# cartographer-project/point_cloud_viewer

Measured on NVIDIA H100. Metric: build_octree Mpoints/sec, higher is better.
Workload: dtype f64

## Files before the change

point_cloud_viewer_b200/csrc/build_host.hpp:

```cpp
#pragma once
#include <algorithm>
#include <chrono>
#include <cmath>
#include <cstdint>
#include <cstdio>
#include <cstdlib>
#include <cstring>
#include <stdexcept>
#include <string>
#include <vector>

#include "chain.h"

namespace pcv {

typedef unsigned __int128 u128;

struct PointsView {
    const double* x;
    const double* y;
    const double* z;
    uint64_t stride;
    const uint8_t* rgb;
    const float* intensity;
// ... 84 lines not shown
    uint64_t arena_used;
    uint32_t deepest_level, pad;
    uint32_t nleaves, place_tiles;
    uint64_t out_points, xyz_bytes, algo_xyz;
    PassState pass[kMaxPasses + 1];
};
enum : int32_t { kErrHistMismatch = 1, kErrTooDeep = 2, kErrCapacity = 3 };

struct ShardSpec {
    int k = 0;
    const uint64_t* counts = nullptr;
    PCV_HD static size_t level_offset(int level) { return (((size_t)1 << (3 * level)) - 8) / 7; }
    uint64_t count_at(int level, uint64_t index) const { return counts[level_offset(level) + index]; }
};

struct PlanRun {
    uint32_t nodes, actives, tiles, chunks;
    uint64_t next_pts, arena_pts;
};

struct IngestArgs {
    PointsView pts;
    void* rec_out;
    uint32_t* col_out;
    uint8_t* dig_out;
    int G0;
    bool wide;
    uint32_t ntiles;
    LevelTable lv;
    double root_min[3];
};

struct PassArgs {
    int pass, level, G, nbins;
    int Gn;
    bool wide;
    bool rec_has_col;
    bool holes;
    const RemoteBufs* remote;
    const float* int_in;
    double e1, e2, ry2, eb, eh, ryh;
    int enc1, enc2, ench, fast;
    const void* rec_in;
    void* rec_next;
    void* arena;
    const uint32_t* col_in;
    uint32_t* col_next;
    uint32_t* col_arena;
    const uint8_t* dig_in;
    uint8_t* dig_next;
    BuildState* st;
    const ActiveDesc* active;
    ActiveDesc* active_next;
    const ChunkDesc* chunks;
    ChunkDesc* chunks_next;
    uint32_t* tile_active;
    uint32_t* tile_counts;
    uint32_t* chunk_sums;
    uint64_t* node_bins;
    BucketDesc* buckets;
    PlanRun* plan_runs;
    DevNode* nodes;
    int32_t* children;
    uint32_t cap_active, cap_nodes, cap_tiles, cap_chunks;
    uint64_t max_points;
    double resolution;
    int shard_k;
    const uint64_t* shard_counts;
    LevelTable lv;
};

struct PlaceArgs {
    bool wide;
    PointsView pts;
    const void* arena;
    const uint32_t* col_arena;
    int fast;
    const DNode* d_nodes;
    const uint32_t* d_leaf_tile_begin;
    const uint32_t* d_leaf_node;
    uint32_t nleaves;
    uint32_t ntiles;
    uint64_t npoints, xyz_bytes;
    uint32_t prefetch_tiles = 0;
    uint8_t* out_xyz;
    uint8_t* out_rgb;
    float* out_intensity;
    uint32_t* out_src;
};

PCV_HD uint32_t upper_index(const uint32_t* begin, size_t stride_words, uint32_t n, uint32_t b) {
    uint32_t lo = 0, hi = n;
    while (hi - lo > 1) {
        const uint32_t mid = (lo + hi) >> 1;
        if (begin[(size_t)mid * stride_words] <= b)
            lo = mid;
        else
            hi = mid;
    }
    return lo;
}
PCV_HD TileDesc tile_of(const ActiveDesc* active, uint32_t nactive, uint32_t b) {
    const uint32_t i = upper_index(&active[0].tile_begin, sizeof(ActiveDesc) / 4, nactive, b);
    const ActiveDesc& act = active[i];
    const uint64_t o = (uint64_t)(b - act.tile_begin) * kTilePoints;
    const uint64_t rem = act.count - o;
    return TileDesc{act.start + o, (uint32_t)(rem < kTilePoints ? rem : kTilePoints), i};
}
PCV_HD LeafTile leaf_tile_of(const PlaceArgs& a, uint32_t b) {
    const uint32_t l = upper_index(a.d_leaf_tile_begin, 1, a.nleaves, b);
    const uint32_t node = a.d_leaf_node[l];
    const DNode& nd = a.d_nodes[node];
    const uint64_t o = (uint64_t)(b - a.d_leaf_tile_begin[l]) * kPlaceTile;
    const uint64_t rem = nd.count - o;
    return LeafTile{nd.arena_off + o, o, node, (uint32_t)(rem < kPlaceTile ? rem : kPlaceTile)};
}

template <bool EMIT>
PCV_HD void plan_active(const PassArgs& a, uint32_t ai, PlanRun& run, int32_t& err, uint32_t& deepest) {
    const ActiveDesc act = a.active[ai];
    const DevNode pn = a.nodes[act.node];
    const uint64_t* nb = a.node_bins + (size_t)ai * a.nbins;
    BucketDesc* bk = a.buckets + (size_t)ai * a.nbins;
    const int w = a.nbins / 8;
    uint32_t nlocal = 0;
    if (!EMIT) {
        uint64_t total = 0;
        for (int b = 0; b < a.nbins; ++b) total += nb[b];
        if (total != act.count) err = kErrHistMismatch;
    }
    auto route = [&](uint32_t node_index, int level, const double m[3], uint64_t cnt, bool split, int b0, int b1, int keep) {
        BucketDesc bd{};
        bd.b0 = (uint16_t)b0;
        bd.b1 = (uint16_t)b1;
        bd.keep = (uint8_t)keep;
        if (split) {
            bd.kind = 0;
            bd.dest = run.next_pts;
            const uint32_t nt = (uint32_t)((cnt + kTilePoints - 1) / kTilePoints);
            const uint32_t nc = (nt + kChunkTiles - 1) / kChunkTiles;
            if (EMIT && run.actives < a.cap_active && run.chunks + nc <= a.cap_chunks) {
                ActiveDesc& na = a.active_next[run.actives];
                na.m[0] = m[0], na.m[1] = m[1], na.m[2] = m[2];
                na.e = a.lv.edge[level];
                na.start = run.next_pts;
                na.count = cnt;
                na.chunk_begin = run.chunks;
                na.nchunks = nc;
                na.tile_begin = run.tiles;
                na.node = node_index;
                for (uint32_t o = 0, c = 0; o < nt; o += kChunkTiles, ++c)
                    a.chunks_next[run.chunks + c] = ChunkDesc{run.tiles + o, (nt - o < kChunkTiles ? nt - o : kChunkTiles), run.actives, o == 0 ? 1u : 0u};
            }
            run.actives += 1;
            run.tiles += nt;
            run.chunks += nc;
            run.next_pts += cnt;
        } else {
            bd.kind = 1;
            bd.dest = run.arena_pts;
            if (EMIT && node_index < a.cap_nodes) a.nodes[node_index].arena_off = run.arena_pts;
            run.arena_pts += cnt;
            if (a.holes) run.next_pts += cnt;
            if ((uint32_t)level > deepest) deepest = (uint32_t)level;
        }
        if (EMIT) bk[nlocal] = bd;
        ++nlocal;
// ... 637 lines not shown
    r.enc = lv.enc[0];
    r.count = total;
    nodes.push_back(r);
    for (size_t i = 0; i < nodes.size(); ++i) {
        if (nodes[i].level >= k - 1) continue;
        for (int c = 0; c < 8; ++c) {
            const HNode p = nodes[i];
            const uint64_t cidx = ((uint64_t)p.index << 3) + (uint64_t)c;
            const uint64_t cnt = sp.count_at(p.level + 1, cidx);
            if (cnt == 0) continue;
            HNode x{};
            x.level = p.level + 1;
            x.index = cidx;
            x.parent = (int)i;
            for (int q = 0; q < 8; ++q) x.child[q] = -1;
            x.count = cnt;
            x.e = lv.edge[x.level];
            x.m[0] = (c & 4) ? p.m[0] + x.e : p.m[0];
            x.m[1] = (c & 2) ? p.m[1] + x.e : p.m[1];
            x.m[2] = (c & 1) ? p.m[2] + x.e : p.m[2];
            x.enc = lv.enc[x.level];
            nodes[i].child[c] = (int)nodes.size();
            nodes.push_back(x);
        }
    }
    std::vector<uint64_t> unit_off(nodes.size() * 8, 0);
    for (size_t i = nodes.size(); i-- > 0;) {
        HNode& x = nodes[i];
        uint64_t off = 0;
        if (x.level == k - 1) {
            for (int c = 0; c < 8; ++c) {
                unit_off[i * 8 + c] = off;
                off += (unit_nsub[((uint64_t)x.index << 3) + (uint64_t)c] + 7) / 8;
            }
        } else {
            for (int c = 0; c < 8; ++c) {
                if (x.child[c] < 0) continue;
                nodes[x.child[c]].off_in_parent = off;
                off += (nodes[x.child[c]].n_sub + 7) / 8;
            }
        }
        x.n_sub = off;
    }
    for (auto& x : nodes) x.final_count = x.parent < 0 ? x.n_sub : x.n_sub - (x.n_sub + 7) / 8;
    R.sorted.resize(nodes.size());
    for (size_t i = 0; i < nodes.size(); ++i) R.sorted[i] = (int)i;
    std::sort(R.sorted.begin(), R.sorted.end(), [&](int a, int b) {
        if (nodes[a].level != nodes[b].level) return nodes[a].level < nodes[b].level;
        return nodes[a].index < nodes[b].index;
    });
    uint64_t poff = 0, boff = 0, arena_total = 0;
    for (int i : R.sorted) {
        HNode& x = nodes[i];
        x.out_point_off = poff;
        boff = (boff + 15) & ~15ull;
        x.out_xyz_off = boff;
        poff += x.final_count;
        boff += x.final_count * 3 * (uint64_t)enc_bytes(x.enc);
        if (x.level == k - 1) {
            x.arena_off = arena_total;
            arena_total += x.n_sub;
        }
    }
    if (arena_total != npoints || poff != npoints) throw BuildError(-1, "top assembly: gathered point count does not match the unit sizes");
    R.xyz_bytes = boff;

    const int cenc = lv.enc[k - 1], bpc = enc_bytes(cenc);
    const size_t rec_bytes = wide ? sizeof(RecW) : sizeof(RecN);
    std::vector<uint8_t> recs((size_t)npoints * rec_bytes);
    std::vector<uint32_t> cols(npoints);
    for (uint64_t i = 0; i < npoints; ++i) {
        uint64_t c[3] = {0, 0, 0};
        for (int a = 0; a < 3; ++a) std::memcpy(&c[a], xyz + (i * 3 + a) * bpc, (size_t)bpc);
        if (wide) {
            RecW w{{c[0], c[1], c[2]}, (uint32_t)i, 0};
            std::memcpy(&recs[i * rec_bytes], &w, sizeof w);
        } else {
            RecN w{{(uint32_t)c[0], (uint32_t)c[1], (uint32_t)c[2]}, (uint32_t)i};
            std::memcpy(&recs[i * rec_bytes], &w, sizeof w);
        }
        cols[i] = (uint32_t)rgb[3 * i] | ((uint32_t)rgb[3 * i + 1] << 8) | ((uint32_t)rgb[3 * i + 2] << 16);
    }
    std::vector<void*> scratch;
    auto up = [&](const void* h, size_t bytes) {
        void* d = be.dmalloc(bytes ? bytes : 16);
        scratch.push_back(d);
        if (bytes) be.h2d(d, h, bytes);
        return d;
    };
    std::vector<DNode> dn(nodes.size());
    std::vector<uint32_t> leaf_tile_begin, leaf_node;
    uint32_t nplace_tiles = 0;
    for (size_t i = 0; i < nodes.size(); ++i) {
        const HNode& x = nodes[i];
        DNode& d = dn[i];
        for (int a = 0; a < 3; ++a) d.m[a] = x.m[a];
        d.e = x.e;
        d.ry = 1.0 / x.e;
        d.off_in_parent = x.off_in_parent;
        d.out_point_off = x.out_point_off;
        d.out_xyz_off = x.out_xyz_off;
        d.arena_off = x.arena_off;
        d.count = x.level == k - 1 ? x.n_sub : 0;
        d.parent = x.parent;
        d.enc = x.enc;
        if (x.level == k - 1 && x.n_sub) {
            leaf_tile_begin.push_back(nplace_tiles);
            leaf_node.push_back((uint32_t)i);
            nplace_tiles += (uint32_t)((x.n_sub + kPlaceTile - 1) / kPlaceTile);
        }
    }
    leaf_tile_begin.push_back(nplace_tiles);
    PlaceArgs pl{};
    pl.wide = wide;
    pl.pts = PointsView{nullptr, nullptr, nullptr, 1, nullptr, intensity ? (const float*)up(intensity, (size_t)npoints * 4) : nullptr, npoints};
    pl.arena = up(recs.data(), recs.size());
    pl.col_arena = (const uint32_t*)up(cols.data(), cols.size() * 4);
    pl.fast = lv.fast;
    pl.d_nodes = (const DNode*)up(dn.data(), dn.size() * sizeof(DNode));
    pl.d_leaf_tile_begin = (const uint32_t*)up(leaf_tile_begin.data(), leaf_tile_begin.size() * 4);
    pl.d_leaf_node = (const uint32_t*)up(leaf_node.data(), leaf_node.size() * 4);
    pl.nleaves = (uint32_t)leaf_node.size();
    pl.ntiles = nplace_tiles;
    pl.npoints = npoints;
    pl.xyz_bytes = boff;
    R.d_xyz = (uint8_t*)be.dmalloc(boff + 32);
    R.d_rgb = (uint8_t*)be.dmalloc(std::max<uint64_t>(npoints * 3, 16));
    R.d_src = (uint32_t*)be.dmalloc(std::max<uint64_t>(npoints * 4, 16));
    R.d_intensity = intensity ? (float*)be.dmalloc(std::max<uint64_t>(npoints * 4, 16)) : nullptr;
    pl.out_xyz = R.d_xyz;
    pl.out_rgb = R.d_rgb;
    pl.out_intensity = R.d_intensity;
    pl.out_src = R.d_src;
    be.place(pl);
    for (void* p : scratch) be.dfree(p);
    return R;
}

}
```

point_cloud_viewer_b200/csrc/kernels_build.cuh:

```cuda
#pragma once
#include <cuda_runtime.h>

#include <map>
#include <type_traits>
#include <unordered_map>

#include "build_host.hpp"
#include "chain_device.cuh"

namespace pcv {

#define PCV_CUDA_CHECK(x)                                                                            \
    do {                                                                                             \
        cudaError_t e_ = (x);                                                                        \
        if (e_ != cudaSuccess) throw ::pcv::BuildError(-2, std::string("CUDA: ") + cudaGetErrorString(e_) + " at " #x); \
    } while (0)

__device__ __forceinline__ double warp_min(double v) {
#pragma unroll
    for (int o = 16; o > 0; o >>= 1) v = fmin(v, __shfl_xor_sync(0xffffffffu, v, o));
    return v;
}
__device__ __forceinline__ double warp_max(double v) {
#pragma unroll
    for (int o = 16; o > 0; o >>= 1) v = fmax(v, __shfl_xor_sync(0xffffffffu, v, o));
    return v;
}

__global__ void __launch_bounds__(256) k_bbox(PointsView p, double* __restrict__ partial) {
    double mn[3] = {INFINITY, INFINITY, INFINITY}, mx[3] = {-INFINITY, -INFINITY, -INFINITY};
    const uint64_t step = (uint64_t)gridDim.x * blockDim.x;
    uint64_t i = (uint64_t)blockIdx.x * blockDim.x + threadIdx.x;
    const uint64_t s = p.stride;
    for (; i + 3 * step < p.n; i += 4 * step) {
        double vx[4], vy[4], vz[4];
#pragma unroll
        for (int u = 0; u < 4; ++u) {
            vx[u] = __ldg(p.x + (i + u * step) * s);
            vy[u] = __ldg(p.y + (i + u * step) * s);
            vz[u] = __ldg(p.z + (i + u * step) * s);
        }
#pragma unroll
        for (int u = 0; u < 4; ++u) {
            mn[0] = fmin(mn[0], vx[u]);
            mx[0] = fmax(mx[0], vx[u]);
            mn[1] = fmin(mn[1], vy[u]);
            mx[1] = fmax(mx[1], vy[u]);
            mn[2] = fmin(mn[2], vz[u]);
            mx[2] = fmax(mx[2], vz[u]);
        }
    }
    for (; i < p.n; i += step) {
        double x = __ldg(p.x + i * s), y = __ldg(p.y + i * s), z = __ldg(p.z + i * s);
        mn[0] = fmin(mn[0], x);
        mx[0] = fmax(mx[0], x);
        mn[1] = fmin(mn[1], y);
        mx[1] = fmax(mx[1], y);
        mn[2] = fmin(mn[2], z);
        mx[2] = fmax(mx[2], z);
    }
    __shared__ double sh[8][6];
    const int w = threadIdx.x >> 5, l = threadIdx.x & 31;
#pragma unroll
    for (int a = 0; a < 3; ++a) {
        double lo = warp_min(mn[a]), hi = warp_max(mx[a]);
        if (l == 0) {
            sh[w][a] = lo;
            sh[w][3 + a] = hi;
        }
    }
    __syncthreads();
    if (threadIdx.x < 6) {
        double v = sh[0][threadIdx.x];
        for (int k = 1; k < 8; ++k) v = threadIdx.x < 3 ? fmin(v, sh[k][threadIdx.x]) : fmax(v, sh[k][threadIdx.x]);
        partial[blockIdx.x * 6 + threadIdx.x] = v;
    }
}

__device__ __forceinline__ void l2_prefetch(const void* p, uint64_t bytes) {
    const uintptr_t b = (reinterpret_cast<uintptr_t>(p) + 15) & ~(uintptr_t)15;
    const uintptr_t e = (reinterpret_cast<uintptr_t>(p) + bytes) & ~(uintptr_t)15;
    if (e > b) asm volatile("cp.async.bulk.prefetch.L2.global [%0], %1;" ::"l"(b), "r"((uint32_t)(e - b)) : "memory");
}
template <bool WIDE>
struct RecT;
template <>
struct RecT<false> {
    typedef RecN type;
};
template <>
struct RecT<true> {
    typedef RecW type;
};

template <bool WIDE>
__device__ __forceinline__ void load_rec(const void* base, uint64_t i, uint64_t c[3], uint32_t& idx) {
    if (WIDE) {
        const ulonglong2* p = reinterpret_cast<const ulonglong2*>(base) + 2 * i;
        const ulonglong2 v0 = __ldg(p), v1 = __ldg(p + 1);
        c[0] = v0.x;
        c[1] = v0.y;
        c[2] = v1.x;
        idx = (uint32_t)v1.y;
    } else {
        const uint4 v = __ldg(reinterpret_cast<const uint4*>(base) + i);
        c[0] = v.x;
        c[1] = v.y;
        c[2] = v.z;
        idx = v.w;
    }
}
template <bool WIDE>
__device__ __forceinline__ void store_rec(void* base, uint64_t i, const uint64_t c[3], uint32_t idx) {
    if (WIDE) {
        ulonglong2 v0, v1;
        v0.x = c[0];
        v0.y = c[1];
        v1.x = c[2];
        v1.y = idx;
        ulonglong2* p = reinterpret_cast<ulonglong2*>(base) + 2 * i;
        p[0] = v0;
        p[1] = v1;
    } else {
        uint4 v;
        v.x = (uint32_t)c[0];
        v.y = (uint32_t)c[1];
        v.z = (uint32_t)c[2];
        v.w = idx;
        reinterpret_cast<uint4*>(base)[i] = v;
    }
}

__device__ __forceinline__ uint32_t smem_u32(const void* p) { return (uint32_t)__cvta_generic_to_shared(p); }
__device__ __forceinline__ void mbar_init(uint64_t* bar, uint32_t count) {
    asm volatile("mbarrier.init.shared.b64 [%0], %1;" ::"r"(smem_u32(bar)), "r"(count) : "memory");
    asm volatile("fence.mbarrier_init.release.cluster;" ::: "memory");
}
__device__ __forceinline__ void mbar_expect_tx(uint64_t* bar, uint32_t bytes) {
    asm volatile("mbarrier.arrive.expect_tx.release.cta.shared::cta.b64 _, [%0], %1;" ::"r"(smem_u32(bar)), "r"(bytes) : "memory");
}
__device__ __forceinline__ void tma_bulk_load(void* smem_dst, const void* gmem_src, uint32_t bytes, uint64_t* bar) {
    asm volatile("cp.async.bulk.shared::cluster.global.mbarrier::complete_tx::bytes [%0], [%1], %2, [%3];" ::"r"(smem_u32(smem_dst)), "l"(gmem_src), "r"(bytes),
                 "r"(smem_u32(bar))
                 : "memory");
}
__device__ __forceinline__ void mbar_wait(uint64_t* bar, uint32_t parity) {
    uint32_t done = 0;
    while (!done) {
        asm volatile(
            "{\n\t.reg .pred P;\n\t"
            "mbarrier.try_wait.parity.shared::cta.b64 P, [%1], %2;\n\t"
            "selp.b32 %0, 1, 0, P;\n\t}"
            : "=r"(done)
            : "r"(smem_u32(bar)), "r"(parity)
            : "memory");
    }
}

template <bool WIDE>
__device__ __forceinline__ void smem_load_rec(const unsigned char* srec, uint32_t i, uint64_t c[3], uint32_t& idx) {
    if (WIDE) {
        const ulonglong2* p = reinterpret_cast<const ulonglong2*>(srec) + 2 * (size_t)i;
        const ulonglong2 v0 = p[0], v1 = p[1];
        c[0] = v0.x, c[1] = v0.y, c[2] = v1.x, idx = (uint32_t)v1.y;
    } else {
        const uint4 v = reinterpret_cast<const uint4*>(srec)[i];
        c[0] = v.x, c[1] = v.y, c[2] = v.z, idx = v.w;
    }
}

constexpr int kIngestThreads = 256;
constexpr size_t kRgbStage = (size_t)kTilePoints * 3 + 32;

template <bool WIDE, int FAST, int kIngestBatch>
__device__ __forceinline__ unsigned ingest_tile(const IngestArgs& a, uint64_t start, uint32_t count, const uint32_t* scol) {
    unsigned bad = 0;
    const double e0 = a.lv.edge[0], e1 = a.lv.edge[1], ry1 = a.lv.ry[1];
    for (uint32_t i0 = threadIdx.x; i0 < count; i0 += kIngestThreads * kIngestBatch) {
      double qq[kIngestBatch][3];
#pragma unroll
      for (int u = 0; u < kIngestBatch; ++u) {
          const uint32_t i = i0 + u * kIngestThreads;
          const uint64_t g = start + (i < count ? i : i0);
          qq[u][0] = __ldcg(a.pts.x + g * a.pts.stride);
          qq[u][1] = __ldcg(a.pts.y + g * a.pts.stride);
          qq[u][2] = __ldcg(a.pts.z + g * a.pts.stride);
      }
#pragma unroll
      for (int u = 0; u < kIngestBatch; ++u) {
        const uint32_t i = i0 + u * kIngestThreads;
        if (i >= count) break;
        const uint64_t g = start + i;
        double q[3] = {qq[u][0], qq[u][1], qq[u][2]}, m[3] = {a.root_min[0], a.root_min[1], a.root_min[2]};
        if (FAST == 2) bad |= input_bad(q[0]) | input_bad(q[1]) | input_bad(q[2]);
// ... 674 lines not shown
                        pb.dig = (unsigned long long)rb.dig_next + (unsigned long long)first;
                        const long long slot0 = leaf ? first + (long long)(bd.dest >> 32) - (long long)(uint32_t)bd.dest : first;
                        PassBucketExt bx;
                        bx.inten = (unsigned long long)rb.intensity + (unsigned long long)(slot0 * 4);
                        bx.slot0 = (uint32_t)slot0;
                        bx.pad = 0;
                        bext[lb] = bx;
                    } else {
                    pb.rec = (unsigned long long)(leaf ? a.arena : a.rec_next) + (unsigned long long)(first * (long long)recsz);
                    pb.col = (unsigned long long)(leaf ? a.col_arena : a.col_next) + (unsigned long long)(first * 4);
                    pb.dig = (unsigned long long)a.dig_next + (unsigned long long)first;
                    }
                    pb.start = run;
                    pb.kk = (uint32_t)bd.keep | (leaf ? 0x100u : 0u);
                    bdst[lb] = pb;
#pragma unroll
                    for (int w = 0; w < kWarps; ++w) {
                        const uint32_t c = cnt[w * nbmax + lb];
                        cnt[w * nbmax + lb] = run;
                        run += c;
                    }
                }
            }
        }
        __syncthreads();
#pragma unroll
        for (int r = 0; r < kSubRounds; ++r) {
            const uint32_t i = warp * kWarpItems + r * 32 + lane;
            const uint32_t lbv = info[r] & 0xFFFFu, rank = (info[r] >> 16) & 31u, gsize = ((info[r] >> 26) & 31u) + 1u;
            const int leader = (int)((info[r] >> 21) & 31u);
            uint32_t old = 0;
            if (lane == leader && lbv != 0xFFFFu) {
                old = cnt[warp * nbmax + lbv];
                cnt[warp * nbmax + lbv] = old + gsize;
            }
            old = __shfl_sync(0xffffffffu, old, leader);
            if (lbv != 0xFFFFu) perm[old + rank] = i | (lbv << 12);
            __syncwarp();
        }
        if (stage_next) {
            asm volatile("cp.async.wait_all;" ::: "memory");
            pass_make_desc(&descs[s ^ 1u], ntile, *snact, nact);
            pass_stage_small<WIDE>(a, descs[s ^ 1u], smem_raw + PassSmem<WIDE>::off_small + (size_t)(s ^ 1u) * PassSmem<WIDE>::small_bytes, &mbar[s ^ 1u]);
        }
        __syncthreads();
        mbar_wait(&mbar[2], it & 1u);
        if (FASTMODE == 1) {
            const unsigned bad = pass_finish<WIDE, 1, REMOTE, ENCU>(a, pt, srec, scol, sdig, perm, bdst, bext);
            if (__syncthreads_or((int)bad)) pass_finish<WIDE, 0, REMOTE, ENCU>(a, pt, srec, scol, sdig, perm, bdst, bext);
        } else {
            pass_finish<WIDE, FASTMODE, REMOTE, ENCU>(a, pt, srec, scol, sdig, perm, bdst, bext);
        }
        __syncthreads();
        if (stage_next) pass_stage_big<WIDE>(a, descs[s ^ 1u], smem_raw, &mbar[2]);
    }
}

__device__ __forceinline__ void store_code(uint8_t* p, uint64_t c, int enc) {
    if (enc == ENC_U8)
        *p = (uint8_t)c;
    else if (enc == ENC_U16)
        *reinterpret_cast<uint16_t*>(p) = (uint16_t)c;
    else if (enc == ENC_F32)
        *reinterpret_cast<uint32_t*>(p) = (uint32_t)c;
    else
        *reinterpret_cast<uint64_t*>(p) = c;
}

__device__ __forceinline__ void place_store(const PlaceArgs& a, const DNode& nd, uint64_t slot, const uint64_t c[3], uint32_t col, uint32_t idx) {
    const uint64_t dp = nd.out_point_off + slot;
    const int bpc = enc_bytes(nd.enc);
    uint8_t* px = a.out_xyz + nd.out_xyz_off + slot * 3 * (uint64_t)bpc;
    store_code(px, c[0], nd.enc);
    store_code(px + bpc, c[1], nd.enc);
    store_code(px + 2 * bpc, c[2], nd.enc);
    uint8_t* rd = a.out_rgb + 3ull * dp;
    rd[0] = (uint8_t)col;
    rd[1] = (uint8_t)(col >> 8);
    rd[2] = (uint8_t)(col >> 16);
    a.out_src[dp] = idx;
    if (a.out_intensity) a.out_intensity[dp] = __ldg(a.pts.intensity + idx);
}

template <bool WIDE, int ENC, int FAST>
__device__ __forceinline__ unsigned place_stayers(const PlaceArgs& a, const LeafTile& lt, const DNode& nd) {
    unsigned bad = 0;
    const uint32_t nst = lt.count - (lt.count + 7) / 8;
    for (uint32_t s = threadIdx.x; s < nst; s += blockDim.x) {
        const uint32_t i = 8 * (s / 7) + (s % 7) + 1;
        uint64_t c[3];
        uint32_t idx;
        load_rec<WIDE>(a.arena, lt.arena_start + i, c, idx);
        const uint32_t col = __ldg(a.col_arena + lt.arena_start + i);
#pragma unroll
        for (int k = 0; k < 3; ++k) c[k] = encode_axis<ENC, FAST>(decode_axis<ENC>(c[k], nd.m[k], nd.e), nd.m[k], nd.e, nd.ry, bad);
        if (!FAST || !bad) {
            const uint64_t j = lt.j0 + i;
            place_store(a, nd, j - (j >> 3) - 1, c, col, idx);
        }
    }
    return bad;
}

template <bool WIDE>
__device__ __forceinline__ void place_movers(const PlaceArgs& a, const LeafTile& lt, const DNode& leaf, bool all_points) {
    const uint32_t step = all_points ? 1u : 8u;
    for (uint32_t i = threadIdx.x * step; i < lt.count; i += blockDim.x * step) {
        uint64_t c[3];
        uint32_t idx;
        load_rec<WIDE>(a.arena, lt.arena_start + i, c, idx);
        const uint32_t col = __ldg(a.col_arena + lt.arena_start + i);
        uint64_t j = lt.j0 + i;
        DNode nd = leaf;
        while (nd.parent >= 0 && (j & 7) == 0) {
            const DNode P = a.d_nodes[nd.parent];
#pragma unroll
            for (int k = 0; k < 3; ++k) {
                if (a.fast) {
                    const double q = decode1_fast(c[k], nd.m[k], nd.e, nd.enc);
                    c[k] = encode1_fast(q, P.m[k], P.e, P.ry, P.enc);
                } else {
                    const double q = decode1(c[k], nd.m[k], nd.e, nd.enc);
                    c[k] = encode1(q, P.m[k], P.e, P.enc);
                }
            }
            j = nd.off_in_parent + (j >> 3);
            nd = P;
        }
        uint64_t slot = j;
        if (nd.parent >= 0) {
#pragma unroll
            for (int k = 0; k < 3; ++k) {
                if (a.fast) {
                    const double q = decode1_fast(c[k], nd.m[k], nd.e, nd.enc);
                    c[k] = encode1_fast(q, nd.m[k], nd.e, nd.ry, nd.enc);
                } else {
                    const double q = decode1(c[k], nd.m[k], nd.e, nd.enc);
                    c[k] = encode1(q, nd.m[k], nd.e, nd.enc);
                }
            }
            slot = j - (j >> 3) - 1;
        }
        place_store(a, nd, slot, c, col, idx);
    }
}

template <bool WIDE>
__global__ void __launch_bounds__(256) k_place(const __grid_constant__ PlaceArgs a) {
    const LeafTile lt = leaf_tile_of(a, blockIdx.x);
    const DNode leaf = a.d_nodes[lt.node];
    if (threadIdx.x == 32 && a.prefetch_tiles) {
        const uint64_t first = lt.arena_start + (uint64_t)a.prefetch_tiles * kPlaceTile;
        if (first < a.npoints) {
            const uint64_t cnt = min((uint64_t)kPlaceTile, a.npoints - first), rb = WIDE ? 32 : 16;
            l2_prefetch(reinterpret_cast<const unsigned char*>(a.arena) + first * rb, cnt * rb);
            l2_prefetch(a.col_arena + first, cnt * 4);
        }
    }
    const bool generic = leaf.parent < 0 || (lt.j0 & 7) != 0;
    if (generic) {
        place_movers<WIDE>(a, lt, leaf, true);
        return;
    }
    if (a.fast == 3) {
        PCV_ENC_SWITCH(leaf.enc, place_stayers<WIDE, ENC, 3>(a, lt, leaf);)
    } else if (a.fast) {
        unsigned bad = 0;
        if (a.fast == 2) {
            PCV_ENC_SWITCH(leaf.enc, bad = place_stayers<WIDE, ENC, 2>(a, lt, leaf);)
        } else {
            PCV_ENC_SWITCH(leaf.enc, bad = place_stayers<WIDE, ENC, 1>(a, lt, leaf);)
        }
        if (__syncthreads_or((int)bad)) {
            PCV_ENC_SWITCH(leaf.enc, place_stayers<WIDE, ENC, 0>(a, lt, leaf);)
        }
    } else {
        PCV_ENC_SWITCH(leaf.enc, place_stayers<WIDE, ENC, 0>(a, lt, leaf);)
    }
    place_movers<WIDE>(a, lt, leaf, false);
}

struct CudaBackend : Backend {
    cudaStream_t stream = nullptr;
    uint64_t launches = 0;
    cudaEvent_t ev[4] = {nullptr, nullptr, nullptr, nullptr};
    enum { K_BBOX = 0, K_INGEST, K_DIGHIST, K_SCAN, K_PLAN, K_PASS, K_PLACE, K_PLY, K_COUNT };
    struct KStat {
        uint64_t launches = 0, bytes = 0;
        double ms = 0;
    };
    bool profile = false;
    KStat kstat[K_COUNT];
    struct Pending {
        int k;
        cudaEvent_t e0, e1;
        uint64_t bytes;
        int pass;
    };
    std::vector<Pending> pending;
    void prof_begin(int k, uint64_t bytes, int pass = -1) {
        if (!profile) return;
        Pending p{k, nullptr, nullptr, bytes, pass};
        cudaEventCreate(&p.e0);
        cudaEventCreate(&p.e1);
        cudaEventRecord(p.e0, stream);
        pending.push_back(p);
    }
    void prof_end() {
        if (!profile) return;
        cudaEventRecord(pending.back().e1, stream);
    }
    void prof_collect() {
        for (auto& p : pending) {
            float ms = 0;
            cudaEventElapsedTime(&ms, p.e0, p.e1);
            kstat[p.k].launches++;
            kstat[p.k].ms += ms;
            kstat[p.k].bytes += p.bytes;
            cudaEventDestroy(p.e0);
            cudaEventDestroy(p.e1);
        }
        pending.clear();
    }
    void prof_reset() {
        for (auto& k : kstat) k = KStat();
    }

    explicit CudaBackend(cudaStream_t s) : stream(s) {
        for (auto& e : ev) PCV_CUDA_CHECK(cudaEventCreate(&e));
        allow_smem_all();
    }
    ~CudaBackend() override {
        cache_release();
        if (ev_back) cudaEventDestroy(ev_back);
        for (auto& b : back_chunks) cudaFreeHost(b.p);
        for (auto& e : ev)
            if (e) cudaEventDestroy(e);
        if (pin) cudaFreeHost(pin);
        if (pin_back) cudaFreeHost(pin_back);
    }
    static constexpr size_t kCacheMin = (size_t)1 << 20;
    struct CachedBlock {
        void* p;
        uint64_t seq;
    };
    std::unordered_map<void*, size_t> big_live;
    std::multimap<size_t, CachedBlock> big_free;
    size_t cached_bytes = 0, cache_cap = 0;
    uint64_t cache_seq = 0;
    void cache_release() {
        for (auto& kv : big_free) cudaFreeAsync(kv.second.p, stream);
        big_free.clear();
        cached_bytes = 0;
    }
    void cache_evict_oldest() {
        auto best = big_free.begin();
        for (auto it = big_free.begin(); it != big_free.end(); ++it)
            if (it->second.seq < best->second.seq) best = it;
        cudaFreeAsync(best->second.p, stream);
        cached_bytes -= best->first;
        big_free.erase(best);
    }
// ... 17 lines not shown
            auto it = big_free.find(bytes);
            if (it != big_free.end()) {
                p = it->second.p;
                big_free.erase(it);
                cached_bytes -= bytes;
                big_live[p] = bytes;
                return p;
            }
        }
        cudaError_t e = cudaMallocAsync(&p, bytes ? bytes : 16, stream);
        if (e == cudaErrorMemoryAllocation && !big_free.empty()) {
            cudaGetLastError();
            cache_release();
            e = cudaMallocAsync(&p, bytes ? bytes : 16, stream);
        }
        PCV_CUDA_CHECK(e);
        if (bytes >= kCacheMin) big_live[p] = bytes;
        return p;
    }
    void dfree(void* p) override {
        if (!p) return;
        auto it = big_live.find(p);
        if (it == big_live.end()) {
            cudaFreeAsync(p, stream);
            return;
        }
        if (!cache_cap) {
            size_t fr = 0, tot = 0;
            cudaMemGetInfo(&fr, &tot);
            cache_cap = tot / 2;
        }
        const size_t bytes = it->second;
        big_live.erase(it);
        big_free.emplace(bytes, CachedBlock{p, ++cache_seq});
        cached_bytes += bytes;
        while (cached_bytes > cache_cap && !big_free.empty()) cache_evict_oldest();
    }
    uint8_t* pin = nullptr;
    size_t pin_cap = 0, pin_off = 0;
    void h2d(void* d, const void* h, size_t bytes) override {
        if (bytes == 0) return;
        const size_t need = (bytes + 255) & ~(size_t)255;
        if (need > pin_cap / 2) {
            PCV_CUDA_CHECK(cudaStreamSynchronize(stream));
            if (pin) cudaFreeHost(pin);
            pin_cap = std::max<size_t>(need * 4, (size_t)64 << 20);
            PCV_CUDA_CHECK(cudaMallocHost(&pin, pin_cap));
            pin_off = 0;
        }
        if (pin_off + need > pin_cap) {
            PCV_CUDA_CHECK(cudaStreamSynchronize(stream));
            pin_off = 0;
        }
        std::memcpy(pin + pin_off, h, bytes);
        PCV_CUDA_CHECK(cudaMemcpyAsync(d, pin + pin_off, bytes, cudaMemcpyHostToDevice, stream));
        pin_off += need;
    }
    uint8_t* pin_back = nullptr;
    size_t pin_back_cap = 0;
    void d2h(void* h, const void* d, size_t bytes) override {
        if (bytes > pin_back_cap) {
            if (pin_back) cudaFreeHost(pin_back);
            pin_back_cap = std::max<size_t>(bytes * 2, (size_t)8 << 20);
            PCV_CUDA_CHECK(cudaMallocHost(&pin_back, pin_back_cap));
        }
        PCV_CUDA_CHECK(cudaMemcpyAsync(pin_back, d, bytes, cudaMemcpyDeviceToHost, stream));
        PCV_CUDA_CHECK(cudaStreamSynchronize(stream));
        std::memcpy(h, pin_back, bytes);
        pin_off = 0;
    }
    void mark(int what) override { cudaEventRecord(ev[what], stream); }

    void zero(void* d, size_t bytes) override {
        if (bytes) PCV_CUDA_CHECK(cudaMemsetAsync(d, 0, bytes, stream));
    }
    static void allow_smem_all() {
        for (int w = 0; w < 2; ++w)
            for (int r = 0; r < 2; ++r)
                for (int f = 0; f < 4; ++f)
                    for (int e = -1; e <= ENC_F32; ++e) {
                        const void* fn = pass_kernel(w != 0, r != 0, f, e);
                        if (fn) cudaFuncSetAttribute(fn, cudaFuncAttributeMaxDynamicSharedMemorySize, (int)(w ? PassSmem<true>::bytes : PassSmem<false>::bytes));
                    }
    }
    int sms = 0;
    bool no_prefetch = false;
    int sm_count() {
        if (!sms) {
            int dev = 0;
            cudaGetDevice(&dev);
            cudaDeviceGetAttribute(&sms, cudaDevAttrMultiProcessorCount, dev);
            no_prefetch = std::getenv("PCV_NO_PREFETCH") != nullptr;
        }
        return sms;
    }
    uint32_t resident(int blocks_per_sm) { return (sm_count(), no_prefetch) ? 0u : (uint32_t)(sms * blocks_per_sm); }

    void ingest(const IngestArgs& a) override {
        const uint32_t grid = std::min<uint32_t>(a.ntiles, (uint32_t)sm_count() * 32u);
        const uint64_t rec = a.wide ? sizeof(RecW) : sizeof(RecN);
        prof_begin(K_INGEST, a.pts.n * (27 + rec + 4 + 1));
        static const int batch = std::getenv("PCV_INGEST_BATCH") ? std::atoi(std::getenv("PCV_INGEST_BATCH")) : 2;
#define PCV_INGEST(W, F)                                                 \
    if (batch == 1)                                                      \
        k_ingest<W, F, 1><<<grid, kIngestThreads, 0, stream>>>(a);      \
    else                                                                 \
        k_ingest<W, F, 2><<<grid, kIngestThreads, 0, stream>>>(a)
        switch ((a.wide ? 4 : 0) + a.lv.fast) {
            case 0: PCV_INGEST(false, 0); break;
            case 1: PCV_INGEST(false, 1); break;
            case 2: PCV_INGEST(false, 2); break;
            case 3: PCV_INGEST(false, 3); break;
            case 4: PCV_INGEST(true, 0); break;
            case 5: PCV_INGEST(true, 1); break;
            case 6: PCV_INGEST(true, 2); break;
            default: PCV_INGEST(true, 3); break;
        }
#undef PCV_INGEST
        prof_end();
        ++launches;
        PCV_CUDA_CHECK(cudaGetLastError());
    }
    void pass(const PassArgs& a) override {
        hist_scan_launch(a);
        plan_launch(a);
        partition_launch(a);
        launches += 9;
        pass_wide = a.wide;
        PCV_CUDA_CHECK(cudaGetLastError());
    }
    void plan_launch(const PassArgs& a) {
        const int nsm = sm_count();
        prof_begin(K_PLAN, 0, a.pass);
        const uint32_t pg = std::min<uint32_t>((a.cap_active + kPlanNodeThreads - 1) / kPlanNodeThreads, (uint32_t)nsm * 8u);
        k_plan_count<<<pg, kPlanNodeThreads, 0, stream>>>(a);
        k_plan_scan<<<1, kPlanThreads, 0, stream>>>(a);
        k_plan_emit<<<pg, kPlanNodeThreads, 0, stream>>>(a);
        prof_end();
    }
    void finish_plan(const FinishArgs& f_in, int last_level) override {
        FinishArgs f = f_in;
        prof_begin(K_PLAN, 0);
        for (int L = last_level; L >= 0; --L) {
            f.level = L;
            k_sub_level<<<sm_count() * 2, 256, 0, stream>>>(f);
        }
        k_sub_layout<<<1, kPlanThreads, 0, stream>>>(f);
        prof_end();
        launches += (uint64_t)last_level + 2;
        PCV_CUDA_CHECK(cudaGetLastError());
    }
    struct BackChunk {
        uint8_t* p;
        size_t cap, off;
    };
    std::vector<BackChunk> back_chunks;
    cudaEvent_t ev_back = nullptr;
    const void* d2h_begin(const void* d, size_t bytes) override {
        const size_t need = ((bytes ? bytes : 1) + 255) & ~(size_t)255;
        BackChunk* c = nullptr;
        for (auto& b : back_chunks)
            if (b.off + need <= b.cap) {
                c = &b;
                break;
            }
        if (!c) {
            BackChunk nb{nullptr, std::max<size_t>(need, (size_t)32 << 20), 0};
            PCV_CUDA_CHECK(cudaMallocHost(&nb.p, nb.cap));
            back_chunks.push_back(nb);
            c = &back_chunks.back();
        }
        uint8_t* dst = c->p + c->off;
        c->off += need;
        if (bytes) PCV_CUDA_CHECK(cudaMemcpyAsync(dst, d, bytes, cudaMemcpyDeviceToHost, stream));
        if (!ev_back) PCV_CUDA_CHECK(cudaEventCreateWithFlags(&ev_back, cudaEventDisableTiming));
        PCV_CUDA_CHECK(cudaEventRecord(ev_back, stream));
        return dst;
    }
    void d2h_wait() override {
        if (ev_back) PCV_CUDA_CHECK(cudaEventSynchronize(ev_back));
        for (auto& b : back_chunks) b.off = 0;
    }
    void plan(const PassArgs& a) override {
        plan_launch(a);
        launches += 3;
        PCV_CUDA_CHECK(cudaGetLastError());
    }
    template <bool W, bool R, int E>
    static const void* pass_kernel_f(int fast) {
        switch (fast) {
            case 0: return (const void*)k_pass<W, R, 0, E>;
            case 1: return (const void*)k_pass<W, R, 1, E>;
            case 2: return (const void*)k_pass<W, R, 2, E>;
            default: return (const void*)k_pass<W, R, 3, E>;
        }
    }
    static const void* pass_kernel(bool wide, bool remote, int fast, int encu) {
        if (wide) return encu >= 0 ? nullptr : (remote ? pass_kernel_f<true, true, -1>(fast) : pass_kernel_f<true, false, -1>(fast));
        if (remote) return encu >= 0 ? nullptr : pass_kernel_f<false, true, -1>(fast);
        switch (encu) {
            case ENC_U8: return pass_kernel_f<false, false, ENC_U8>(fast);
            case ENC_U16: return pass_kernel_f<false, false, ENC_U16>(fast);
            case ENC_F32: return pass_kernel_f<false, false, ENC_F32>(fast);
            default: return pass_kernel_f<false, false, -1>(fast);
        }
    }
    void partition_launch(const PassArgs& a) {
        const int nsm = sm_count();
        prof_begin(K_PASS, 0, a.pass);
        const uint32_t gw = std::min<uint32_t>(a.cap_tiles, (uint32_t)(nsm * PassCfg<true>::blocks_per_sm));
        const uint32_t gn = std::min<uint32_t>(a.cap_tiles, (uint32_t)(nsm * PassCfg<false>::blocks_per_sm));
        int encu = a.enc1;
        if (a.G == 2 && a.enc2 != encu) encu = -1;
        if (a.Gn > 0 && a.ench != encu) encu = -1;
        if (a.wide || a.remote || encu == ENC_F64 || std::getenv("PCV_PASS_GENERIC")) encu = -1;
        const void* fn = pass_kernel(a.wide, a.remote != nullptr, a.fast, encu);
        PassArgs arg = a;
        void* params[1] = {&arg};
        PCV_CUDA_CHECK(cudaLaunchKernel(fn, dim3(a.wide ? gw : gn), dim3(a.wide ? PassCfg<true>::threads : PassCfg<false>::threads), params,
                                        a.wide ? PassSmem<true>::bytes : PassSmem<false>::bytes, stream));
        prof_end();
    }
    void partition(const PassArgs& a) {
        partition_launch(a);
        ++launches;
        pass_wide = a.wide;
        PCV_CUDA_CHECK(cudaGetLastError());
    }
    void hist_scan_launch(const PassArgs& a) {
        const int nsm = sm_count();
        const int th = a.nbins < 32 ? 32 : a.nbins;
        prof_begin(K_DIGHIST, 0, a.pass);
        k_tile_index<<<std::min<uint32_t>(a.cap_chunks, 1024u), 256, 0, stream>>>(a);
        k_dighist<<<nsm * 8, kDigThreads, 0, stream>>>(a);
        prof_end();
        prof_begin(K_SCAN, 0, a.pass);
        k_scan_chunk_sums<<<std::min<uint32_t>(a.cap_chunks, 2048u), th, 0, stream>>>(a);
        k_scan_nodes<<<std::min<uint32_t>(a.cap_active, 2048u), th, 0, stream>>>(a);
        k_scan_tiles<<<std::min<uint32_t>(a.cap_chunks, 2048u), th, 0, stream>>>(a);
        prof_end();
    }
    void hist_scan(const PassArgs& a) override {
        hist_scan_launch(a);
        launches += 5;
        PCV_CUDA_CHECK(cudaGetLastError());
    }
    bool pass_wide = false;
    void pass_points(int pass, uint64_t npoints, uint64_t leaf_points) override {
        const uint64_t rec = pass_wide ? sizeof(RecW) : sizeof(RecN);
        for (auto& p : pending) {
            if (p.pass != pass || p.bytes != 0) continue;
            if (p.k == K_DIGHIST) p.bytes = npoints;
            if (p.k == K_SCAN) p.bytes = (npoints / kTilePoints + 1) * 64 * 12;
            if (p.k == K_PASS) p.bytes = npoints * (rec + 4 + 1) + (npoints - leaf_points) * (rec + 4 + 1) + leaf_points * (rec + 4);
        }
    }
    void place(const PlaceArgs& a_in) override {
        if (a_in.ntiles == 0) return;
        PlaceArgs a = a_in;
        a.prefetch_tiles = resident(4);
        prof_begin(K_PLACE, a.npoints * ((a.wide ? sizeof(RecW) : sizeof(RecN)) + 3 + 3 + 4 + (a.out_intensity ? 8 : 0)) + a.xyz_bytes);
        if (a.wide)
            k_place<true><<<a.ntiles, 256, 0, stream>>>(a);
        else
            k_place<false><<<a.ntiles, 256, 0, stream>>>(a);
        prof_end();
        ++launches;
        PCV_CUDA_CHECK(cudaGetLastError());
    }

    void bbox(const PointsView& p, double mn[3], double mx[3]) {
        if (p.n == 0) {
            for (int a = 0; a < 3; ++a) mn[a] = mx[a] = 0.0;
            return;
        }
        int dev = 0, sms = 132;
        cudaGetDevice(&dev);
        cudaDeviceGetAttribute(&sms, cudaDevAttrMultiProcessorCount, dev);
        const int blocks = (int)std::min<uint64_t>((uint64_t)sms * 8, (p.n + 255) / 256);
        double* d = (double*)dmalloc((size_t)blocks * 6 * 8);
        prof_begin(K_BBOX, p.n * 24);
        k_bbox<<<blocks, 256, 0, stream>>>(p, d);
        prof_end();
        ++launches;
        PCV_CUDA_CHECK(cudaGetLastError());
        std::vector<double> h((size_t)blocks * 6);
        d2h(h.data(), d, h.size() * 8);
        dfree(d);
        for (int a = 0; a < 3; ++a) {
            mn[a] = h[a];
            mx[a] = h[3 + a];
        }
        for (int b = 1; b < blocks; ++b)
            for (int a = 0; a < 3; ++a) {
                mn[a] = std::fmin(mn[a], h[(size_t)b * 6 + a]);
                mx[a] = std::fmax(mx[a], h[(size_t)b * 6 + 3 + a]);
            }
    }
};

}
```

Before: 8472.

## Stage place-kernel tile records into shared memory via TMA bulk copies

The place kernel now bulk-loads each tile's records and colors into shared memory with TMA and an mbarrier, replacing per-thread __ldg loads and the L2 prefetch of future tiles. A small pre-kernel builds a per-block LeafTile table so each block skips the binary search in leaf_tile_of. The leaf node is copied into shared memory, and the parent walk uses pointers instead of copying DNode structs. The cost is an extra launch plus allocation per call, and dynamic shared memory use that may limit occupancy.

```diff
diff --git a/point_cloud_viewer_b200/csrc/build_host.hpp b/point_cloud_viewer_b200/csrc/build_host.hpp
--- a/point_cloud_viewer_b200/csrc/build_host.hpp
+++ b/point_cloud_viewer_b200/csrc/build_host.hpp
@@ -190,7 +190,7 @@
     uint32_t nleaves;
     uint32_t ntiles;
     uint64_t npoints, xyz_bytes;
-    uint32_t prefetch_tiles = 0;
+    const LeafTile* tiles = nullptr;
     uint8_t* out_xyz;
     uint8_t* out_rgb;
     float* out_intensity;
@@ -994,8 +994,8 @@
         cols[i] = (uint32_t)rgb[3 * i] | ((uint32_t)rgb[3 * i + 1] << 8) | ((uint32_t)rgb[3 * i + 2] << 16);
     }
     std::vector<void*> scratch;
-    auto up = [&](const void* h, size_t bytes) {
-        void* d = be.dmalloc(bytes ? bytes : 16);
+    auto up = [&](const void* h, size_t bytes, size_t slack = 0) {
+        void* d = be.dmalloc((bytes ? bytes : 16) + slack);
         scratch.push_back(d);
         if (bytes) be.h2d(d, h, bytes);
         return d;
@@ -1027,7 +1027,7 @@
     pl.wide = wide;
     pl.pts = PointsView{nullptr, nullptr, nullptr, 1, nullptr, intensity ? (const float*)up(intensity, (size_t)npoints * 4) : nullptr, npoints};
     pl.arena = up(recs.data(), recs.size());
-    pl.col_arena = (const uint32_t*)up(cols.data(), cols.size() * 4);
+    pl.col_arena = (const uint32_t*)up(cols.data(), cols.size() * 4, 64);
     pl.fast = lv.fast;
     pl.d_nodes = (const DNode*)up(dn.data(), dn.size() * sizeof(DNode));
     pl.d_leaf_tile_begin = (const uint32_t*)up(leaf_tile_begin.data(), leaf_tile_begin.size() * 4);
diff --git a/point_cloud_viewer_b200/csrc/kernels_build.cuh b/point_cloud_viewer_b200/csrc/kernels_build.cuh
--- a/point_cloud_viewer_b200/csrc/kernels_build.cuh
+++ b/point_cloud_viewer_b200/csrc/kernels_build.cuh
@@ -77,11 +77,6 @@
     }
 }
 
-__device__ __forceinline__ void l2_prefetch(const void* p, uint64_t bytes) {
-    const uintptr_t b = (reinterpret_cast<uintptr_t>(p) + 15) & ~(uintptr_t)15;
-    const uintptr_t e = (reinterpret_cast<uintptr_t>(p) + bytes) & ~(uintptr_t)15;
-    if (e > b) asm volatile("cp.async.bulk.prefetch.L2.global [%0], %1;" ::"l"(b), "r"((uint32_t)(e - b)) : "memory");
-}
 template <bool WIDE>
 struct RecT;
 template <>
@@ -93,23 +88,6 @@
     typedef RecW type;
 };
 
-template <bool WIDE>
-__device__ __forceinline__ void load_rec(const void* base, uint64_t i, uint64_t c[3], uint32_t& idx) {
-    if (WIDE) {
-        const ulonglong2* p = reinterpret_cast<const ulonglong2*>(base) + 2 * i;
-        const ulonglong2 v0 = __ldg(p), v1 = __ldg(p + 1);
-        c[0] = v0.x;
-        c[1] = v0.y;
-        c[2] = v1.x;
-        idx = (uint32_t)v1.y;
-    } else {
-        const uint4 v = __ldg(reinterpret_cast<const uint4*>(base) + i);
-        c[0] = v.x;
-        c[1] = v.y;
-        c[2] = v.z;
-        idx = v.w;
-    }
-}
 template <bool WIDE>
 __device__ __forceinline__ void store_rec(void* base, uint64_t i, const uint64_t c[3], uint32_t idx) {
     if (WIDE) {
@@ -950,16 +928,38 @@
     if (a.out_intensity) a.out_intensity[dp] = __ldg(a.pts.intensity + idx);
 }
 
+template <bool WIDE>
+struct PlaceSmem {
+    static constexpr size_t rec_bytes = WIDE ? 32 : 16;
+    static constexpr size_t off_col = (size_t)kPlaceTile * rec_bytes;
+    static constexpr size_t off_bar = off_col + ((size_t)kPlaceTile + 4) * 4;
+    static constexpr size_t off_node = off_bar + 16;
+    static constexpr size_t bytes = off_node + sizeof(DNode);
+    static_assert(off_col % 16 == 0 && off_bar % 16 == 0 && sizeof(DNode) % 4 == 0, "bulk copy destinations 16-byte aligned, the node copied in whole words");
+};
+static_assert(4 * (PlaceSmem<false>::bytes + 1024) <= 233472, "four narrow place blocks must fit one SM (228 KB, 1 KB reserved per block)");
+
+__global__ void k_place_tiles(const __grid_constant__ PlaceArgs a, LeafTile* __restrict__ tiles) {
+    const uint32_t l = blockIdx.x;
+    const uint32_t t0 = a.d_leaf_tile_begin[l], nt = a.d_leaf_tile_begin[l + 1] - t0;
+    const uint32_t node = a.d_leaf_node[l];
+    const uint64_t arena_off = a.d_nodes[node].arena_off, count = a.d_nodes[node].count;
+    for (uint32_t t = threadIdx.x; t < nt; t += blockDim.x) {
+        const uint64_t o = (uint64_t)t * kPlaceTile, rem = count - o;
+        tiles[t0 + t] = LeafTile{arena_off + o, o, node, (uint32_t)(rem < kPlaceTile ? rem : kPlaceTile)};
+    }
+}
+
 template <bool WIDE, int ENC, int FAST>
-__device__ __forceinline__ unsigned place_stayers(const PlaceArgs& a, const LeafTile& lt, const DNode& nd) {
+__device__ __forceinline__ unsigned place_stayers(const PlaceArgs& a, const LeafTile& lt, const DNode& nd, const unsigned char* srec, const uint32_t* scol) {
     unsigned bad = 0;
     const uint32_t nst = lt.count - (lt.count + 7) / 8;
     for (uint32_t s = threadIdx.x; s < nst; s += blockDim.x) {
         const uint32_t i = 8 * (s / 7) + (s % 7) + 1;
         uint64_t c[3];
         uint32_t idx;
-        load_rec<WIDE>(a.arena, lt.arena_start + i, c, idx);
-        const uint32_t col = __ldg(a.col_arena + lt.arena_start + i);
+        smem_load_rec<WIDE>(srec, i, c, idx);
+        const uint32_t col = scol[i];
 #pragma unroll
         for (int k = 0; k < 3; ++k) c[k] = encode_axis<ENC, FAST>(decode_axis<ENC>(c[k], nd.m[k], nd.e), nd.m[k], nd.e, nd.ry, bad);
         if (!FAST || !bad) {
@@ -971,81 +971,91 @@
 }
 
 template <bool WIDE>
-__device__ __forceinline__ void place_movers(const PlaceArgs& a, const LeafTile& lt, const DNode& leaf, bool all_points) {
+__device__ __forceinline__ void place_movers(const PlaceArgs& a, const LeafTile& lt, const DNode& leaf, bool all_points, const unsigned char* srec,
+                                             const uint32_t* scol) {
     const uint32_t step = all_points ? 1u : 8u;
     for (uint32_t i = threadIdx.x * step; i < lt.count; i += blockDim.x * step) {
         uint64_t c[3];
         uint32_t idx;
-        load_rec<WIDE>(a.arena, lt.arena_start + i, c, idx);
-        const uint32_t col = __ldg(a.col_arena + lt.arena_start + i);
+        smem_load_rec<WIDE>(srec, i, c, idx);
+        const uint32_t col = scol[i];
         uint64_t j = lt.j0 + i;
-        DNode nd = leaf;
-        while (nd.parent >= 0 && (j & 7) == 0) {
-            const DNode P = a.d_nodes[nd.parent];
+        const DNode* nd = &leaf;
+        while (nd->parent >= 0 && (j & 7) == 0) {
+            const DNode* P = a.d_nodes + nd->parent;
 #pragma unroll
             for (int k = 0; k < 3; ++k) {
                 if (a.fast) {
-                    const double q = decode1_fast(c[k], nd.m[k], nd.e, nd.enc);
-                    c[k] = encode1_fast(q, P.m[k], P.e, P.ry, P.enc);
+                    const double q = decode1_fast(c[k], nd->m[k], nd->e, nd->enc);
+                    c[k] = encode1_fast(q, P->m[k], P->e, P->ry, P->enc);
                 } else {
-                    const double q = decode1(c[k], nd.m[k], nd.e, nd.enc);
-                    c[k] = encode1(q, P.m[k], P.e, P.enc);
+                    const double q = decode1(c[k], nd->m[k], nd->e, nd->enc);
+                    c[k] = encode1(q, P->m[k], P->e, P->enc);
                 }
             }
-            j = nd.off_in_parent + (j >> 3);
+            j = nd->off_in_parent + (j >> 3);
             nd = P;
         }
         uint64_t slot = j;
-        if (nd.parent >= 0) {
+        if (nd->parent >= 0) {
 #pragma unroll
             for (int k = 0; k < 3; ++k) {
                 if (a.fast) {
-                    const double q = decode1_fast(c[k], nd.m[k], nd.e, nd.enc);
-                    c[k] = encode1_fast(q, nd.m[k], nd.e, nd.ry, nd.enc);
+                    const double q = decode1_fast(c[k], nd->m[k], nd->e, nd->enc);
+                    c[k] = encode1_fast(q, nd->m[k], nd->e, nd->ry, nd->enc);
                 } else {
-                    const double q = decode1(c[k], nd.m[k], nd.e, nd.enc);
-                    c[k] = encode1(q, nd.m[k], nd.e, nd.enc);
+                    const double q = decode1(c[k], nd->m[k], nd->e, nd->enc);
+                    c[k] = encode1(q, nd->m[k], nd->e, nd->enc);
                 }
             }
             slot = j - (j >> 3) - 1;
         }
-        place_store(a, nd, slot, c, col, idx);
+        place_store(a, *nd, slot, c, col, idx);
     }
 }
 
 template <bool WIDE>
 __global__ void __launch_bounds__(256) k_place(const __grid_constant__ PlaceArgs a) {
-    const LeafTile lt = leaf_tile_of(a, blockIdx.x);
-    const DNode leaf = a.d_nodes[lt.node];
-    if (threadIdx.x == 32 && a.prefetch_tiles) {
-        const uint64_t first = lt.arena_start + (uint64_t)a.prefetch_tiles * kPlaceTile;
-        if (first < a.npoints) {
-            const uint64_t cnt = min((uint64_t)kPlaceTile, a.npoints - first), rb = WIDE ? 32 : 16;
-            l2_prefetch(reinterpret_cast<const unsigned char*>(a.arena) + first * rb, cnt * rb);
-            l2_prefetch(a.col_arena + first, cnt * 4);
-        }
-    }
+    constexpr size_t recsz = PlaceSmem<WIDE>::rec_bytes;
+    extern __shared__ __align__(128) unsigned char smem_raw[];
+    uint64_t* bar = reinterpret_cast<uint64_t*>(smem_raw + PlaceSmem<WIDE>::off_bar);
+    const LeafTile lt = a.tiles[blockIdx.x];
+    const uint32_t coff = (uint32_t)(lt.arena_start & 3);
+    if (threadIdx.x == 0) {
+        const uint32_t rec_bytes = lt.count * (uint32_t)recsz, col_bytes = ((coff + lt.count) * 4u + 15u) & ~15u;
+        mbar_init(bar, 1);
+        mbar_expect_tx(bar, rec_bytes + col_bytes);
+        tma_bulk_load(smem_raw, reinterpret_cast<const unsigned char*>(a.arena) + lt.arena_start * recsz, rec_bytes, bar);
+        tma_bulk_load(smem_raw + PlaceSmem<WIDE>::off_col, a.col_arena + (lt.arena_start - coff), col_bytes, bar);
+    }
+    DNode* snode = reinterpret_cast<DNode*>(smem_raw + PlaceSmem<WIDE>::off_node);
+    if (threadIdx.x < sizeof(DNode) / 4) reinterpret_cast<uint32_t*>(snode)[threadIdx.x] = reinterpret_cast<const uint32_t*>(a.d_nodes + lt.node)[threadIdx.x];
+    const DNode& leaf = *snode;
+    const unsigned char* srec = smem_raw;
+    const uint32_t* scol = reinterpret_cast<const uint32_t*>(smem_raw + PlaceSmem<WIDE>::off_col) + coff;
+    __syncthreads();
+    mbar_wait(bar, 0);
     const bool generic = leaf.parent < 0 || (lt.j0 & 7) != 0;
     if (generic) {
-        place_movers<WIDE>(a, lt, leaf, true);
+        place_movers<WIDE>(a, lt, leaf, true, srec, scol);
         return;
     }
     if (a.fast == 3) {
-        PCV_ENC_SWITCH(leaf.enc, place_stayers<WIDE, ENC, 3>(a, lt, leaf);)
+        PCV_ENC_SWITCH(leaf.enc, place_stayers<WIDE, ENC, 3>(a, lt, leaf, srec, scol);)
     } else if (a.fast) {
         unsigned bad = 0;
         if (a.fast == 2) {
-            PCV_ENC_SWITCH(leaf.enc, bad = place_stayers<WIDE, ENC, 2>(a, lt, leaf);)
+            PCV_ENC_SWITCH(leaf.enc, bad = place_stayers<WIDE, ENC, 2>(a, lt, leaf, srec, scol);)
         } else {
-            PCV_ENC_SWITCH(leaf.enc, bad = place_stayers<WIDE, ENC, 1>(a, lt, leaf);)
+            PCV_ENC_SWITCH(leaf.enc, bad = place_stayers<WIDE, ENC, 1>(a, lt, leaf, srec, scol);)
         }
         if (__syncthreads_or((int)bad)) {
-            PCV_ENC_SWITCH(leaf.enc, place_stayers<WIDE, ENC, 0>(a, lt, leaf);)
+            PCV_ENC_SWITCH(leaf.enc, place_stayers<WIDE, ENC, 0>(a, lt, leaf, srec, scol);)
         }
     } else {
-        PCV_ENC_SWITCH(leaf.enc, place_stayers<WIDE, ENC, 0>(a, lt, leaf);)
-    }
-    place_movers<WIDE>(a, lt, leaf, false);
+        PCV_ENC_SWITCH(leaf.enc, place_stayers<WIDE, ENC, 0>(a, lt, leaf, srec, scol);)
+    }
+    place_movers<WIDE>(a, lt, leaf, false, srec, scol);
 }
 
 struct CudaBackend : Backend {
@@ -1229,19 +1239,18 @@
                         const void* fn = pass_kernel(w != 0, r != 0, f, e);
                         if (fn) cudaFuncSetAttribute(fn, cudaFuncAttributeMaxDynamicSharedMemorySize, (int)(w ? PassSmem<true>::bytes : PassSmem<false>::bytes));
                     }
+        cudaFuncSetAttribute(k_place<false>, cudaFuncAttributeMaxDynamicSharedMemorySize, (int)PlaceSmem<false>::bytes);
+        cudaFuncSetAttribute(k_place<true>, cudaFuncAttributeMaxDynamicSharedMemorySize, (int)PlaceSmem<true>::bytes);
     }
     int sms = 0;
-    bool no_prefetch = false;
     int sm_count() {
         if (!sms) {
             int dev = 0;
             cudaGetDevice(&dev);
             cudaDeviceGetAttribute(&sms, cudaDevAttrMultiProcessorCount, dev);
-            no_prefetch = std::getenv("PCV_NO_PREFETCH") != nullptr;
         }
         return sms;
     }
-    uint32_t resident(int blocks_per_sm) { return (sm_count(), no_prefetch) ? 0u : (uint32_t)(sms * blocks_per_sm); }
 
     void ingest(const IngestArgs& a) override {
         const uint32_t grid = std::min<uint32_t>(a.ntiles, (uint32_t)sm_count() * 32u);
@@ -1405,15 +1414,18 @@
     void place(const PlaceArgs& a_in) override {
         if (a_in.ntiles == 0) return;
         PlaceArgs a = a_in;
-        a.prefetch_tiles = resident(4);
+        LeafTile* tiles = (LeafTile*)dmalloc((size_t)a.ntiles * sizeof(LeafTile));
+        a.tiles = tiles;
         prof_begin(K_PLACE, a.npoints * ((a.wide ? sizeof(RecW) : sizeof(RecN)) + 3 + 3 + 4 + (a.out_intensity ? 8 : 0)) + a.xyz_bytes);
+        k_place_tiles<<<a.nleaves, 128, 0, stream>>>(a, tiles);
         if (a.wide)
-            k_place<true><<<a.ntiles, 256, 0, stream>>>(a);
+            k_place<true><<<a.ntiles, 256, PlaceSmem<true>::bytes, stream>>>(a);
         else
-            k_place<false><<<a.ntiles, 256, 0, stream>>>(a);
+            k_place<false><<<a.ntiles, 256, PlaceSmem<false>::bytes, stream>>>(a);
         prof_end();
-        ++launches;
+        launches += 2;
         PCV_CUDA_CHECK(cudaGetLastError());
+        dfree(tiles);
     }
 
     void bbox(const PointsView& p, double mn[3], double mx[3]) {
```

After: 8873 (median of 6 runs). 1.05x the previous value.
